# ecmwf-ifs/dwarf-p-cloudsc2-tl-ad

Measured on AMD Instinct MI355X. Metric: CLOUDSC2 NL columns/sec (fp64, NLEV=137), higher is better.
Workload: dtype f64

## Files before the change

### dwarf_p_cloudsc2_tl_ad_amd/__init__.py

```python
from . import binding
from .binding import (Cloudsc2Error, Params, adjoint_verdict, default_params, device_available, get_math_mode,
                      set_math_mode, taylor_verdict)
from .state import (Cloudsc2State, bytes_per_column, ceta_from_table, column_range, nblocks_of, random_table,
                    state_from_table, synthetic_table, validate_l1)
from .driver import (DeviceState, FlatFields, ResidentState, cloudsc_driver, cloudsc_driver_ad, cloudsc_driver_tl,
                     run_state)
from .autograd import PARAM_NAMES, Cloudsc2Outputs, cloudsc2, param_jacobian, satur
```

### dwarf_p_cloudsc2_tl_ad_amd/binding.py

```python
from __future__ import annotations

import ctypes as C
import os

import numpy as np

CLOUDSC2_MAX_NLEV = 200
CLOUDSC2_EINVAL, CLOUDSC2_ENODEVICE, CLOUDSC2_ETLWRONG = -1, -2, -3

_HERE = os.path.dirname(os.path.abspath(__file__))
SINGLE = os.environ.get("CLOUDSC2_PRECISION", "double").strip().lower() in ("single", "sp", "f32", "fp32", "float32")
REAL = np.float32 if SINGLE else np.float64
REAL_BYTES = 4 if SINGLE else 8
c_real = C.c_float if SINGLE else C.c_double
LIB_PATH = os.environ.get("CLOUDSC2_LIB") or os.path.join(_HERE, "csrc", "libcloudsc2_hip_sp.so" if SINGLE else "libcloudsc2_hip.so")


def torch_real():
    import torch

    return torch.float32 if SINGLE else torch.float64


class Cloudsc2Error(RuntimeError):
# ... 17 lines not shown

    def set_ceta(self, ceta) -> "Params":
        ceta = np.asarray(ceta, dtype=np.float64)
        if ceta.size > CLOUDSC2_MAX_NLEV:
            raise ValueError("nlev exceeds CLOUDSC2_MAX_NLEV")
        self.nlev = int(ceta.size)
        for k, v in enumerate(ceta):
            self.ceta[k] = float(v)
        return self

    def ceta_array(self) -> np.ndarray:
        return np.array(self.ceta[: self.nlev], dtype=np.float64)


class Field(C.Structure):

    _fields_ = [("ptr", C.c_void_p), ("block_stride", C.c_longlong)]


IN_NAMES = ("paph", "pap", "q", "qsat", "t", "l", "i", "lude", "lu", "mfu", "mfd", "gtent", "gtenq", "gtenl",
            "gteni", "supsat")
OUT_NAMES = ("tent", "tenq", "tenl", "teni", "clc", "fplsl", "fplsn", "fhpsl", "fhpsn", "covptot")
PARAM_NAMES = ("rkconv", "rclcrit", "rlptrc", "rpecons")


class Inputs(C.Structure):

    _fields_ = [(n, Field) for n in IN_NAMES]


class Outputs(C.Structure):

    _fields_ = [(n, Field) for n in OUT_NAMES]


def _load() -> C.CDLL:
    if not os.path.exists(LIB_PATH):
        raise ImportError(
            f"{LIB_PATH} not found: the HIP library has not been built (run `python -c 'import __graft_entry__ as g; "
            "g.build()'` or `make -C dwarf_p_cloudsc2_tl_ad_amd/csrc`). There is no CPU fallback.")
    try:
        import torch
    except ImportError:
        pass
    lib = C.CDLL(LIB_PATH)
    dp = C.POINTER(C.c_double)
    rp = C.POINTER(c_real)
    pp = C.POINTER(Params)
    lib.cloudsc2_real_bytes.restype = C.c_int
    if lib.cloudsc2_real_bytes() != REAL_BYTES:
        raise ImportError(f"{LIB_PATH} works on {lib.cloudsc2_real_bytes()}-byte reals, CLOUDSC2_PRECISION asks for {REAL_BYTES}")
    lib.cloudsc2_params_default.argtypes = [pp]
    lib.cloudsc2_params_default.restype = None
    lib.cloudsc2_last_error.restype = C.c_char_p
    lib.cloudsc2_device_available.restype = C.c_int
    lib.cloudsc2_set_math_mode.argtypes = [C.c_int]
    lib.cloudsc2_set_math_mode.restype = None
    lib.cloudsc2_get_math_mode.restype = C.c_int
    lib.cloudsc2_nl_launch.argtypes = [pp, C.c_double, C.c_int, C.c_int, C.c_int, C.POINTER(Inputs), C.POINTER(Outputs),
                                       Field, C.c_double, C.c_void_p]
    lib.cloudsc2_satur_launch.argtypes = [pp, C.c_int, C.c_int, C.c_int, Field, Field, Field, C.c_void_p]
    lib.cloudsc2_tl_launch.argtypes = [pp, C.c_double, C.c_int, C.c_int, C.c_int, C.POINTER(Inputs), C.POINTER(Outputs),
                                       C.POINTER(Inputs), C.POINTER(Outputs), C.c_void_p]
    lib.cloudsc2_tl_launch_self.argtypes = [pp, C.c_double, C.c_int, C.c_int, C.c_int, C.POINTER(Inputs), C.POINTER(Outputs), C.c_double,
                                            C.POINTER(Outputs), C.c_void_p, C.c_void_p]
    lib.cloudsc2_ad_launch_reverse_norms.argtypes = [pp, C.c_double, C.c_int, C.c_int, C.c_int, C.POINTER(Inputs), C.POINTER(Outputs),
# ... 23 lines not shown
    lib.cloudsc2_par_work_doubles.argtypes = [C.c_int, C.c_int, C.POINTER(C.c_longlong)]
    lib.cloudsc2_par_work_doubles.restype = C.c_int
    lib.cloudsc2_tl_launch_par.argtypes = [pp, C.c_double, C.c_int, C.c_int, C.c_int, C.c_int, C.POINTER(Inputs), C.POINTER(Inputs),
                                           C.POINTER(C.c_double), C.POINTER(Outputs), C.c_void_p]
    lib.cloudsc2_tl_launch_par.restype = C.c_int
    lib.cloudsc2_vjp_launch_par.argtypes = [pp, C.c_double, C.c_int, C.c_int, C.c_int, C.c_int, C.POINTER(Inputs), C.POINTER(Outputs),
                                            C.POINTER(Inputs), C.POINTER(Outputs), C.c_void_p, C.c_void_p, C.c_void_p, C.c_void_p]
    lib.cloudsc2_vjp_launch_par.restype = C.c_int
    lib.cloudsc2_tl_launch_parjac.argtypes = [pp, C.c_double, C.c_int, C.c_int, C.c_int, C.POINTER(Inputs), C.POINTER(Outputs), C.c_void_p]
    lib.cloudsc2_tl_launch_parjac.restype = C.c_int
    lib.cloudsc2_batch_max.argtypes = []
    lib.cloudsc2_batch_max.restype = C.c_int
    lib.cloudsc2_tl_launch_batch.argtypes = [pp, C.c_double, C.c_int, C.c_int, C.c_int, C.POINTER(Inputs), C.c_int,
                                             C.POINTER(Inputs), C.POINTER(Outputs), C.c_void_p]
    lib.cloudsc2_tl_launch_batch.restype = C.c_int
    lib.cloudsc2_vjp_launch_batch.argtypes = [pp, C.c_double, C.c_int, C.c_int, C.c_int, C.POINTER(Inputs), C.POINTER(Outputs), C.c_int,
                                              C.POINTER(Inputs), C.POINTER(Outputs), C.c_void_p, C.c_void_p]
    lib.cloudsc2_vjp_launch_batch.restype = C.c_int
    lib.cloudsc2_taylor_sums_launch.argtypes = [C.c_int, C.c_int, C.c_int, C.POINTER(Outputs), C.POINTER(Outputs),
                                                C.POINTER(Outputs), C.c_double, C.c_void_p, C.c_void_p]
    lib.cloudsc2_taylor_sweep_work_doubles.argtypes = [C.c_int, C.c_int, C.POINTER(C.c_longlong)]
    lib.cloudsc2_taylor_sweep_work_doubles.restype = C.c_int
    lib.cloudsc2_taylor_sweep_launch.argtypes = [pp, C.c_double, C.c_int, C.c_int, C.c_int, C.c_int, C.POINTER(Inputs), C.POINTER(Outputs),
                                                 C.POINTER(Outputs), C.c_void_p, C.c_void_p, C.c_void_p]
    lib.cloudsc2_taylor_sweep_launch.restype = C.c_int
    lib.cloudsc2_adjoint_norms_launch.argtypes = [C.c_int, C.c_int, C.c_int, C.POINTER(Inputs), C.POINTER(Field),
                                                  C.POINTER(Outputs), C.POINTER(Inputs), C.c_void_p, C.c_void_p,
                                                  C.c_void_p]
    host18 = [rp] * 18
    lib.cloudsc2_nl_run.argtypes = [pp, C.c_int, C.c_int, C.c_int, C.c_double] + host18 + [dp]
    lib.cloudsc2_tl_taylor_run.argtypes = [pp, C.c_int, C.c_int, C.c_int, C.c_double] + host18 + [dp, dp]
    lib.cloudsc2_ad_symmetry_run.argtypes = [pp, C.c_int, C.c_int, C.c_int, C.c_double] + host18 + [dp, dp]
    lib.cloudsc2_release_workspace.restype = None
    lib.cloudsc2_state_create.argtypes = [C.c_int, C.c_int, C.c_int, C.POINTER(C.c_void_p)]
    lib.cloudsc2_state_destroy.argtypes = [C.c_void_p]
    lib.cloudsc2_state_destroy.restype = None
    lib.cloudsc2_state_field.argtypes = [C.c_void_p, C.c_int, C.POINTER(Field)]
    lib.cloudsc2_state_blocking.argtypes = [C.c_void_p, C.POINTER(C.c_int), C.POINTER(C.c_int)]
    lib.cloudsc2_state_blocking.restype = C.c_int
    lib.cloudsc2_state_expand.argtypes = [C.c_void_p, C.c_int, rp, C.c_int, C.c_int, C.c_longlong]
    lib.cloudsc2_state_upload.argtypes = [C.c_void_p] + host18
    lib.cloudsc2_state_download.argtypes = [C.c_void_p] + [rp] * 7
    lib.cloudsc2_state_nl.argtypes = [C.c_void_p, pp, C.c_double, C.c_int, dp]
    lib.cloudsc2_state_tl_taylor.argtypes = [C.c_void_p, pp, C.c_double, dp, dp]
    lib.cloudsc2_state_ad_symmetry.argtypes = [C.c_void_p, pp, C.c_double, dp, dp]
    lib.cloudsc2_state_validate.argtypes = [C.c_void_p, C.c_int, C.c_int, rp, C.c_int, C.c_int, C.c_longlong, dp]
    for name in ("cloudsc2_state_create", "cloudsc2_state_field", "cloudsc2_state_expand", "cloudsc2_state_upload",
                 "cloudsc2_state_download", "cloudsc2_state_nl", "cloudsc2_state_tl_taylor", "cloudsc2_state_ad_symmetry",
                 "cloudsc2_state_validate"):
        getattr(lib, name).restype = C.c_int
    lib.cloudsc2_device_malloc.argtypes = [C.POINTER(C.c_void_p), C.c_size_t]
    lib.cloudsc2_device_free.argtypes = [C.c_void_p]
    lib.cloudsc2_device_malloc_info.argtypes = [C.POINTER(C.c_int), dp, dp, dp]
    lib.cloudsc2_device_malloc_info.restype = None
    lib.cloudsc2_device_malloc_counts.argtypes = [C.POINTER(C.c_longlong), C.POINTER(C.c_longlong)]
    lib.cloudsc2_device_malloc_counts.restype = None
    lib.cloudsc2_pace_plan.argtypes = [C.c_longlong, C.c_longlong, C.POINTER(C.c_int), C.POINTER(C.c_int), C.POINTER(C.c_int)]
    lib.cloudsc2_pace_plan.restype = C.c_int
    lib.cloudsc2_simd_population.argtypes = [C.c_longlong, C.c_int, C.c_longlong, C.c_int, C.POINTER(C.c_int), C.POINTER(C.c_int)]
    lib.cloudsc2_simd_population.restype = C.c_int
    lib.cloudsc2_dispatch_probe.argtypes = [C.POINTER(C.c_longlong), C.POINTER(C.c_longlong)]
    lib.cloudsc2_dispatch_probe.restype = C.c_int
    lib.cloudsc2_pace_probe.argtypes = [C.c_int, C.POINTER(C.c_longlong), C.POINTER(C.c_longlong)]
    lib.cloudsc2_pace_probe.restype = C.c_int
    lib.cloudsc2_synthetic_table.argtypes = [C.c_int, C.c_int, C.c_double, C.c_double, C.c_double] + [C.POINTER(C.c_double)] * 12
    lib.cloudsc2_synthetic_table.restype = C.c_int
# ... 6 lines not shown
    lib.cloudsc2_device_probe.argtypes = [C.c_void_p, C.c_size_t, C.c_int, C.c_int, dp]
    lib.cloudsc2_device_probe.restype = C.c_int
    lib.cloudsc2_device_malloc_state.argtypes = [C.POINTER(C.c_void_p), C.c_size_t, C.c_int, C.c_int, C.c_int]
    lib.cloudsc2_device_malloc_state.restype = C.c_int
    lib.cloudsc2_taylor_verdict.argtypes = [dp, C.POINTER(C.c_int)]
    lib.cloudsc2_adjoint_verdict.argtypes = [C.c_double]
    expand_args = [rp, C.c_int, C.c_int, C.c_longlong, C.c_int, C.c_int, C.c_int, C.c_longlong, Field]
    lib.cloudsc2_expand_launch.argtypes = expand_args + [C.c_void_p]
    lib.cloudsc2_validate_workspace_doubles.restype = C.c_int
    lib.cloudsc2_validate_launch.argtypes = expand_args + [dp, dp, C.c_void_p]
    lib.cloudsc2_expand_offsets.argtypes = [C.c_int, C.c_longlong, C.c_longlong, C.c_int, C.c_int, C.POINTER(C.c_longlong),
                                            C.POINTER(C.c_int)]
    lib.cloudsc2_expand_offsets.restype = None
    lib.cloudsc2_validate_relerr.argtypes = [C.c_double, C.c_double, C.POINTER(C.c_int), C.POINTER(C.c_int)]
    lib.cloudsc2_validate_relerr.restype = C.c_double
    lib.cloudsc2_validate_format.argtypes = [C.c_char_p, C.c_int, dp, C.c_longlong, C.c_char_p, C.c_int]
    lib.cloudsc2_validate_header.argtypes = [C.c_char_p, C.c_int]
    for name in ("cloudsc2_expand_launch", "cloudsc2_validate_launch", "cloudsc2_validate_format", "cloudsc2_validate_header",
                 "cloudsc2_nl_launch", "cloudsc2_satur_launch", "cloudsc2_tl_launch", "cloudsc2_ad_launch",
                 "cloudsc2_taylor_sums_launch", "cloudsc2_adjoint_norms_launch", "cloudsc2_nl_run",
                 "cloudsc2_tl_taylor_run", "cloudsc2_ad_symmetry_run", "cloudsc2_taylor_verdict",
                 "cloudsc2_adjoint_verdict", "cloudsc2_device_malloc", "cloudsc2_device_free"):
        getattr(lib, name).restype = C.c_int
    return lib


lib = _load()

EXPORTED = ("cloudsc2_params_default", "cloudsc2_last_error", "cloudsc2_device_available", "cloudsc2_current_device", "cloudsc2_set_math_mode",
            "cloudsc2_get_math_mode", "cloudsc2_real_bytes", "cloudsc2_nl_launch",
            "cloudsc2_satur_launch", "cloudsc2_satur_lin_launch", "cloudsc2_tl_launch_satur", "cloudsc2_vjp_launch_satur", "cloudsc2_par_work_doubles", "cloudsc2_tl_launch_par", "cloudsc2_vjp_launch_par", "cloudsc2_tl_launch_parjac", "cloudsc2_tl_launch", "cloudsc2_tl_launch_self", "cloudsc2_ad_launch", "cloudsc2_ad_launch_assign",
            "cloudsc2_ad_launch_forward", "cloudsc2_ad_launch_reverse", "cloudsc2_vjp_launch", "cloudsc2_batch_max", "cloudsc2_tl_launch_batch", "cloudsc2_vjp_launch_batch", "cloudsc2_ad_launch_reverse_norms", "cloudsc2_taylor_sums_launch",
            "cloudsc2_taylor_sweep_work_doubles", "cloudsc2_taylor_sweep_launch", "cloudsc2_adjoint_norms_launch", "cloudsc2_nl_run", "cloudsc2_tl_taylor_run", "cloudsc2_ad_symmetry_run",
            "cloudsc2_release_workspace", "cloudsc2_taylor_verdict", "cloudsc2_adjoint_verdict",
            "cloudsc2_expand_launch", "cloudsc2_validate_workspace_doubles", "cloudsc2_validate_launch",
            "cloudsc2_expand_offsets", "cloudsc2_validate_relerr", "cloudsc2_validate_format", "cloudsc2_validate_header",
            "cloudsc2_device_malloc", "cloudsc2_device_free", "cloudsc2_device_malloc_info", "cloudsc2_device_malloc_counts", "cloudsc2_pace_plan", "cloudsc2_simd_population", "cloudsc2_dispatch_probe", "cloudsc2_pace_probe", "cloudsc2_device_prepare", "cloudsc2_device_rules", "cloudsc2_kernel_occupancy", "cloudsc2_device_probe", "cloudsc2_device_malloc_state",
            "cloudsc2_state_create", "cloudsc2_state_destroy", "cloudsc2_state_field", "cloudsc2_state_blocking", "cloudsc2_state_expand",
            "cloudsc2_state_upload", "cloudsc2_state_download", "cloudsc2_state_nl", "cloudsc2_state_tl_taylor",
            "cloudsc2_state_ad_symmetry", "cloudsc2_state_validate", "cloudsc2_synthetic_table")

F_FULL = {"PT": 0, "PQ": 1, "PAP": 2, "PAPH": 3, "PLU": 4, "PLUDE": 5, "PMFU": 6, "PMFD": 7, "PA": 8, "PSUPSAT": 9, "PCOVPTOT": 10,
          "PFPLSL": 11, "PFPLSN": 12, "PFHPSL": 13, "PFHPSN": 14, "QSAT": 15}
F_CML_T, F_LOC_T, F_PCLV_QL = 16, 24, 32


def check(rc: int) -> None:
    if rc != 0:
        raise Cloudsc2Error(rc, (lib.cloudsc2_last_error() or b"").decode())


class DeviceBuffer:

    def __init__(self, nbytes: int, state_geom=None):
        p = C.c_void_p()
        if state_geom is None:
            check(lib.cloudsc2_device_malloc(C.byref(p), int(nbytes)))
        else:
            check(lib.cloudsc2_device_malloc_state(C.byref(p), int(nbytes), *[int(x) for x in state_geom]))
        self.ptr, self.nbytes = int(p.value or 0), int(nbytes)
        self.__cuda_array_interface__ = {"shape": (self.nbytes,), "typestr": "|u1", "data": (self.ptr, False), "version": 2}

    def __del__(self):
        if getattr(self, "ptr", 0):
            lib.cloudsc2_device_free(C.c_void_p(self.ptr))
            self.ptr = 0

# ... 133 lines not shown
```

### dwarf_p_cloudsc2_tl_ad_amd/csrc/cloudsc2_driver.hip

```cpp

#include <thread>
#include "cloudsc2_host.hpp"

using namespace cloudsc2;

namespace {


__global__ void __launch_bounds__(256)
scale_planes_kernel(real_t* dst, long long dst_stride, const real_t* src, long long src_stride, long long plane, long long nblocks,
                    real_t factor) {
  long long i = (long long)blockIdx.x * blockDim.x + threadIdx.x;
  if (i >= plane * nblocks) return;
  long long ibl = i / plane, r = i - ibl * plane;
  dst[ibl * dst_stride + r] = src[ibl * src_stride + r] * factor;
}

__global__ void __launch_bounds__(256)
reblock_kernel(const real_t* __restrict__ src, int np_src, long long stride_src, real_t* __restrict__ dst, int np_dst,
               long long stride_dst, long long nrows, long long ncopy, long long nzero) {
  const long long total = nrows * nzero;
  for (long long e = (long long)blockIdx.x * blockDim.x + threadIdx.x; e < total; e += (long long)gridDim.x * blockDim.x) {
    const long long row = e / nzero, g = e - row * nzero;
    const long long bd = g / np_dst, jd = g - bd * np_dst;
    real_t v = 0;
    if (g < ncopy) {
      const long long bs = g / np_src, js = g - bs * np_src;
      v = src[bs * stride_src + row * np_src + js];
    }
    dst[bd * stride_dst + row * np_dst + jd] = v;
  }
}

constexpr size_t kAlignReals = 256 / sizeof(real_t);
size_t r32(size_t n) { return (n + kAlignReals - 1) & ~(kAlignReals - 1); }
// ... 213 lines not shown
                            &out.covptot};
  for (int k = 0; k < 16; ++k) *fi[k] = fld(base + k * plane, stride);
  for (int k = 0; k < 10; ++k) *fo[k] = fld(base + (16 + k) * plane, stride);
}

size_t flat_in_reals(long long ncols_pad, int nlev) { return 15 * r32((size_t)ncols_pad * nlev) + r32((size_t)ncols_pad * (nlev + 1)); }
size_t flat_out_reals(long long ncols_pad, int nlev) { return 6 * r32((size_t)ncols_pad * nlev) + 4 * r32((size_t)ncols_pad * (nlev + 1)); }

struct Timer {
  hipEvent_t a = nullptr, b = nullptr;
  Timer() = default;
  Timer(const Timer&) = delete;
  Timer& operator=(const Timer&) = delete;
  ~Timer() {
    if (a) (void)hipEventDestroy(a);
    if (b) (void)hipEventDestroy(b);
  }
  int start(hipStream_t st) {
    HIP_TRY(hipEventCreate(&a));
    HIP_TRY(hipEventCreate(&b));
    HIP_TRY(hipEventRecord(a, st));
    return 0;
  }
  int stop(hipStream_t st, double* ms) {
    HIP_TRY(hipEventRecord(b, st));
    HIP_TRY(hipEventSynchronize(b));
    float f = 0;
    HIP_TRY(hipEventElapsedTime(&f, a, b));
    if (ms) *ms = f;
    return 0;
  }
};

struct SlabResources {
  hipStream_t s_up = nullptr, s_k = nullptr;
  std::vector<hipEvent_t> ev;
  SlabResources() = default;
  SlabResources(const SlabResources&) = delete;
  SlabResources& operator=(const SlabResources&) = delete;
  ~SlabResources() {
    for (auto e : ev) if (e) (void)hipEventDestroy(e);
    if (s_up) (void)hipStreamDestroy(s_up);
    if (s_k) (void)hipStreamDestroy(s_k);
  }
  int create(size_t nevents) {
    HIP_TRY(hipStreamCreateWithFlags(&s_up, hipStreamNonBlocking));
    HIP_TRY(hipStreamCreateWithFlags(&s_k, hipStreamNonBlocking));
    ev.assign(nevents, nullptr);
    for (auto& e : ev) HIP_TRY(hipEventCreate(&e));
    return 0;
  }
};

HostState host_view(const HostState& h, long long b0, const DevState& d) {
  const long long S = d.S, H = d.H;
  HostState v = h;
  v.pt += b0 * S; v.pq += b0 * S; v.b_cml += b0 * 8 * S; v.b_loc += b0 * 8 * S; v.pap += b0 * S; v.paph += b0 * H;
  v.plu += b0 * S; v.plude += b0 * S; v.pmfu += b0 * S; v.pmfd += b0 * S; v.pa += b0 * S; v.pclv += b0 * 5 * S;
  v.psupsat += b0 * S; v.pcovptot += b0 * S; v.pfplsl += b0 * H; v.pfplsn += b0 * H; v.pfhpsl += b0 * H; v.pfhpsn += b0 * H;
  return v;
}
DevState dev_view(const DevState& d, long long b0, long long nb) {
  const long long S = d.S, H = d.H;
  DevState v = d;
  v.pt += b0 * S; v.pq += b0 * S; v.b_cml += b0 * 8 * S; v.b_loc += b0 * 8 * S; v.pap += b0 * S; v.paph += b0 * H;
  v.plu += b0 * S; v.plude += b0 * S; v.pmfu += b0 * S; v.pmfd += b0 * S; v.pa += b0 * S; v.pclv += b0 * 5 * S;
  v.psupsat += b0 * S; v.pcovptot += b0 * S; v.pfplsl += b0 * H; v.pfplsn += b0 * H; v.pfhpsl += b0 * H; v.pfhpsn += b0 * H;
  v.qsat += b0 * S;
  v.nblocks = nb;
  return v;
}

int upload_slab_sync(const HostState& h, const DevState& d, long long ncols, int nlev, hipStream_t st) {
  int rc = upload(h, d, ncols, nlev, st);
  if (rc) return rc;
  HIP_TRY(hipStreamSynchronize(st));
  return 0;
}

int nl_run_slabs(const cloudsc2_params* prm, double ptsphy, int nproma, int nlev, int ngptot, const Geom& g, const HostState& h,
                 const DevState& d, double* kernel_ms) {
  const long long nb = d.nblocks;
  const long long slab_blocks = std::max<long long>(1, 16384 / nproma);
  const long long nslabs = (nb + slab_blocks - 1) / slab_blocks;
  int device = 0;
  HIP_TRY(hipGetDevice(&device));
  SlabResources res;
  {
    const int rc_res = res.create((size_t)(2 * nslabs));
    if (rc_res) return rc_res;
  }
  const hipStream_t s_up = res.s_up, s_k = res.s_k;
  const std::vector<hipEvent_t>& ev = res.ev;

  std::atomic<long long> uploaded{0};
  std::atomic<int> up_rc{0};
  std::string up_err;
  auto slab_cols = [&](long long i, long long& b0, long long& nbs, long long& active) {
    b0 = i * slab_blocks;
    nbs = std::min(slab_blocks, nb - b0);
    active = std::min<long long>(nbs * nproma, (long long)ngptot - b0 * nproma);
  };
  std::thread uploader([&] {
    if (hipSetDevice(device) != hipSuccess) { up_rc = CLOUDSC2_EINVAL; up_err = "hipSetDevice failed in the upload thread"; return; }
    for (long long i = 0; i < nslabs && up_rc == 0; ++i) {
      long long b0, nbs, active;
      slab_cols(i, b0, nbs, active);
      int rc = upload_slab_sync(host_view(h, b0, d), dev_view(d, b0, nbs), nbs * nproma, nlev, s_up);
      if (rc) { up_err = g_err; up_rc = rc; return; }
      uploaded.store(i + 1, std::memory_order_release);
    }
  });

  int rc = 0;
  for (long long i = 0; i < nslabs && rc == 0; ++i) {
    while (uploaded.load(std::memory_order_acquire) <= i && up_rc == 0) std::this_thread::yield();
    if (up_rc != 0) break;
    long long b0, nbs, active;
    slab_cols(i, b0, nbs, active);
    const DevState dv = dev_view(d, b0, nbs);
    cloudsc2_inputs in; cloudsc2_outputs out;
    traj_blocks(dv, nproma, nlev, false, in, out);
    if (hipEventRecord(ev[2 * i], s_k) != hipSuccess) { rc = fail(CLOUDSC2_EINVAL, "hipEventRecord failed"); break; }
    rc = cloudsc2_nl_launch(prm, ptsphy, nproma, nlev, (int)active, &in, &out, fld(dv.b_loc + 7LL * nproma * nlev, 8 * dv.S), 0.0, s_k);
    if (rc) break;
    if (hipEventRecord(ev[2 * i + 1], s_k) != hipSuccess) { rc = fail(CLOUDSC2_EINVAL, "hipEventRecord failed"); break; }
    rc = download(host_view(h, b0, d), dv, nbs * nproma, nlev, s_k, nproma, active);
  }
  uploader.join();
  if (rc == 0 && up_rc != 0) rc = fail(up_rc, up_err.c_str());
  const hipError_t e_sync = hipStreamSynchronize(s_k);
  if (rc == 0 && e_sync != hipSuccess) rc = fail(CLOUDSC2_EINVAL, hipGetErrorString(e_sync));
  if (rc == 0 && kernel_ms) {
    double total = 0.0;
    for (long long i = 0; i < nslabs; ++i) {
      float f = 0.f;
      if (hipEventElapsedTime(&f, ev[2 * i], ev[2 * i + 1]) == hipSuccess) total += f;
    }
    *kernel_ms = total;
  }
  (void)g;
  return rc;
}

}

extern "C" {

void cloudsc2_release_workspace(void) {
  std::lock_guard<std::mutex> lock(g_arena_mutex);
  g_arena.release();
}

int cloudsc2_nl_run(const cloudsc2_params* prm, int nproma, int nlev, int ngptot, double ptsphy, const cloudsc2_real* pt,
                    const cloudsc2_real* pq, const cloudsc2_real* b_cml, cloudsc2_real* b_loc, const cloudsc2_real* pap, const cloudsc2_real* paph,
                    const cloudsc2_real* plu, const cloudsc2_real* plude, const cloudsc2_real* pmfu, const cloudsc2_real* pmfd, cloudsc2_real* pa,
                    const cloudsc2_real* pclv, const cloudsc2_real* psupsat, cloudsc2_real* pcovptot, cloudsc2_real* pfplsl, cloudsc2_real* pfplsn,
                    cloudsc2_real* pfhpsl, cloudsc2_real* pfhpsn, double* kernel_ms) {
  Geom g;
  int rc = check_geom(prm, nproma, nlev, ngptot, g);
  if (rc) return rc;
  std::lock_guard<std::mutex> lock(g_arena_mutex);
  const ProbeFn probe = state_probe(nproma, nlev, ngptot);
  if ((rc = g_arena.reserve(state_reals(g.ncols_pad, nlev), &probe, kPlaceOnRequest))) return rc;
  DevState d;
  state_take(g_arena, d, g.ncols_pad, nproma, nlev);
  HostState h = {pt, pq, b_cml, b_loc, pap, paph, plu, plude, pmfu, pmfd, pa, pclv, psupsat, pcovptot, pfplsl, pfplsn, pfhpsl, pfhpsn};
  return nl_run_slabs(prm, ptsphy, nproma, nlev, ngptot, g, h, d, kernel_ms);
}

}
namespace {

size_t taylor_nsums(int ngptot, int nproma_stat) { return (size_t)(((long long)ngptot + nproma_stat - 1) / nproma_stat) * 10 * 2 * 10; }
size_t taylor_ws_reals(long long ncols_pad, int nproma, int nlev, int ngptot, int nproma_stat) {
  (void)nproma;
  const size_t nsums = taylor_nsums(ngptot, nproma_stat);
  return std::max(flat_in_reals(ncols_pad, nlev) + flat_out_reals(ncols_pad, nlev), pair_reals(ncols_pad, nlev)) +
         r32((size_t)(10 * kTaylorLambdas + 10) * (size_t)ncols_pad * kF64) + r32(nsums * kF64);
}
size_t adjoint_ws_reals(long long ncols_pad, int nlev) {
  const size_t ncol = (size_t)ncols_pad;
  return std::max(flat_in_reals(ncols_pad, nlev) + flat_out_reals(ncols_pad, nlev), pair_reals(ncols_pad, nlev)) + r32(ncol * nlev) +
         r32(3 * ncol * kF64) + r32(32 * kF64);
}

int taylor_compute(const cloudsc2_params* prm_in, const Geom& g, int nproma, int nlev, int ngptot, double ptsphy, const DevState& d,
                   Arena& ws, double znormg[10], double* kernel_ms, hipStream_t st, int nproma_stat) {
  const long long nblocks_stat = ((long long)ngptot + nproma_stat - 1) / nproma_stat;
  const size_t nsums = taylor_nsums(ngptot, nproma_stat);
  cloudsc2_inputs inc;
  cloudsc2_outputs tlo;
  pair_take(ws, g.ncols_pad, nproma, nlev, inc, tlo);
  (void)inc;
  double* colsum = ws.take_f64((size_t)(10 * kTaylorLambdas + 10) * (size_t)g.ncols_pad);
  double* sums = ws.take_f64(nsums);
  int rc;
  cloudsc2_inputs in; cloudsc2_outputs out;
  traj_blocks(d, nproma, nlev, true, in, out);
  cloudsc2_params prm_call = *prm_in;
  if (prm_call.math_mode == 0) prm_call.math_mode = 2;
// ... 399 lines not shown
```

### dwarf_p_cloudsc2_tl_ad_amd/driver.py

```python
from __future__ import annotations

import ctypes as C

import numpy as np

from . import binding as B
from .state import PLANE_A, PLANE_Q, PLANE_QI, PLANE_QL, PLANE_QV, PLANE_T, Cloudsc2State, nblocks_of

_dp = C.POINTER(C.c_double)
_rp = C.POINTER(B.c_real)


def _ptr(a: np.ndarray):
    if a.dtype != B.REAL or not a.flags["C_CONTIGUOUS"]:
        raise ValueError(f"state arrays must be C-contiguous {np.dtype(B.REAL).name}")
    return a.ctypes.data_as(_rp)


def _host_args(prm: B.Params, nproma, nlev, ngptot, ptsphy, arrays):
    return [C.byref(prm), int(nproma), int(nlev), int(ngptot), float(ptsphy)] + [_ptr(a) for a in arrays]


def cloudsc_driver(prm: B.Params, numomp, nproma, nlev, ngptot, ngptotg, ptsphy, pt, pq, tendency_cml, tendency_loc, pap,
                   paph, plu, plude, pmfu, pmfd, pa, pclv, psupsat, pcovptot, pfplsl, pfplsn, pfhpsl, pfhpsn) -> float:
    del numomp, ngptotg
    ms = C.c_double(0.0)
    arrays = [pt, pq, tendency_cml, tendency_loc, pap, paph, plu, plude, pmfu, pmfd, pa, pclv, psupsat, pcovptot, pfplsl,
              pfplsn, pfhpsl, pfhpsn]
    B.check(B.lib.cloudsc2_nl_run(*_host_args(prm, nproma, nlev, ngptot, ptsphy, arrays), C.byref(ms)))
    return ms.value


def cloudsc_driver_tl(prm: B.Params, numomp, nproma, nlev, ngptot, ngptotg, ptsphy, pt, pq, tendency_cml, tendency_loc,
                      pap, paph, plu, plude, pmfu, pmfd, pa, pclv, psupsat, pcovptot, pfplsl, pfplsn, pfhpsl, pfhpsn):
    del numomp, ngptotg
    ms = C.c_double(0.0)
    zn = (C.c_double * 10)()
    arrays = [pt, pq, tendency_cml, tendency_loc, pap, paph, plu, plude, pmfu, pmfd, pa, pclv, psupsat, pcovptot, pfplsl,
              pfplsn, pfhpsl, pfhpsn]
    B.check(B.lib.cloudsc2_tl_taylor_run(*_host_args(prm, nproma, nlev, ngptot, ptsphy, arrays), zn, C.byref(ms)))
    znormg = np.array(zn[:], dtype=np.float64)
    ok, itest = B.taylor_verdict(znormg)
    return znormg, ok, itest, ms.value


def cloudsc_driver_ad(prm: B.Params, numomp, nproma, nlev, ngptot, ngptotg, ptsphy, pt, pq, tendency_cml, tendency_loc,
                      pap, paph, plu, plude, pmfu, pmfd, pa, pclv, psupsat, pcovptot, pfplsl, pfplsn, pfhpsl, pfhpsn):
    del numomp, ngptotg
    ms = C.c_double(0.0)
    zn = C.c_double(0.0)
    arrays = [pt, pq, tendency_cml, tendency_loc, pap, paph, plu, plude, pmfu, pmfd, pa, pclv, psupsat, pcovptot, pfplsl,
              pfplsn, pfhpsl, pfhpsn]
    B.check(B.lib.cloudsc2_ad_symmetry_run(*_host_args(prm, nproma, nlev, ngptot, ptsphy, arrays), C.byref(zn), C.byref(ms)))
    return zn.value, B.adjoint_verdict(zn.value), ms.value


def run_state(prm: B.Params, st: Cloudsc2State, which: str = "nl"):
    fn = {"nl": cloudsc_driver, "tl": cloudsc_driver_tl, "ad": cloudsc_driver_ad}[which]
    return fn(prm, 1, st.nproma, st.nlev, st.ngptot, st.ngptot, st.ptsphy, *st.driver_arrays())


def _fld(t, offset_elems: int, stride: int) -> B.Field:
    f = B.Field()
    f.ptr = t.data_ptr() + B.REAL_BYTES * offset_elems
    f.block_stride = stride
    return f


class FlatFields:

    NPLANES = len(B.IN_NAMES) + len(B.OUT_NAMES)

    def __init__(self, kind: str, nb: int, nlev: int, nproma: int, device, zero: bool = True, _views=None, _arena=None):
        self.kind = kind
        names = B.IN_NAMES if kind == "in" else B.OUT_NAMES
        half = {"paph"} if kind == "in" else {"fplsl", "fplsn", "fhpsl", "fhpsn"}
        if _views is not None:
            buf, first = _views
            self.buf = buf
            self.t = {n: buf[:, first + k, : nlev + (1 if n in half else 0), :] for k, n in enumerate(names)}
        else:
            shapes = {n: (nb, nlev + (1 if n in half else 0), nproma) for n in names}
            arena = _arena or B.DeviceArena(B.DeviceArena.size_of(shapes.values(), B.REAL_BYTES), device)
            self.t = {n: arena.take(shp, zero=zero) for n, shp in shapes.items()}
        self.nlev, self.nproma = nlev, nproma

    @classmethod
# ... 335 lines not shown
```

### include/cloudsc2_hip.h

```cpp
#ifndef CLOUDSC2_HIP_H
#define CLOUDSC2_HIP_H

#ifdef __cplusplus
extern "C" {
#endif

#ifdef CLOUDSC2_SINGLE
typedef float cloudsc2_real;
#else
typedef double cloudsc2_real;
#endif

#define CLOUDSC2_MAX_NLEV 200

#define CLOUDSC2_EINVAL    (-1)
#define CLOUDSC2_ENODEVICE (-2)
#define CLOUDSC2_ETLWRONG  (-3)

typedef struct cloudsc2_params {
  double rg, rd, rcpd, retv, rlvtt, rlstt, rlmlt, rtt;
  double r2es, r3les, r3ies, r4les, r4ies, r5les, r5ies, r5alvcp, r5alscp,
         ralvdcp, ralsdcp, rtwat, rtice, rtwat_rtice_r, rvtmp2;
  double rclcrit, rkconv, rlmin, rpecons;
  double rlptrc;
// ... 128 lines not shown
                                double* sums, void* stream);

int cloudsc2_taylor_sweep_work_doubles(int nproma, int ngptot, long long* n);
int cloudsc2_taylor_sweep_launch(const cloudsc2_params* prm, double ptsphy, int nproma, int nlev, int ngptot, int nproma_stat,
                                 const cloudsc2_inputs* in, const cloudsc2_outputs* out, const cloudsc2_outputs* tl,
                                 double* work, double* sums, void* stream);

int cloudsc2_adjoint_norms_launch(int nproma, int nlev, int ngptot, const cloudsc2_inputs* traj_in,
                                  const cloudsc2_field* qsat, const cloudsc2_outputs* y,
                                  const cloudsc2_inputs* x_adj, double* norms, double* blockmax, void* stream);

int cloudsc2_nl_run(const cloudsc2_params* prm, int nproma, int nlev, int ngptot, double ptsphy,
                    const cloudsc2_real* pt, const cloudsc2_real* pq, const cloudsc2_real* b_cml, cloudsc2_real* b_loc,
                    const cloudsc2_real* pap, const cloudsc2_real* paph, const cloudsc2_real* plu, const cloudsc2_real* plude,
                    const cloudsc2_real* pmfu, const cloudsc2_real* pmfd, cloudsc2_real* pa, const cloudsc2_real* pclv,
                    const cloudsc2_real* psupsat, cloudsc2_real* pcovptot, cloudsc2_real* pfplsl, cloudsc2_real* pfplsn,
                    cloudsc2_real* pfhpsl, cloudsc2_real* pfhpsn, double* kernel_ms);

int cloudsc2_tl_taylor_run(const cloudsc2_params* prm, int nproma, int nlev, int ngptot, double ptsphy,
                           const cloudsc2_real* pt, const cloudsc2_real* pq, const cloudsc2_real* b_cml, cloudsc2_real* b_loc,
                           const cloudsc2_real* pap, const cloudsc2_real* paph, const cloudsc2_real* plu, const cloudsc2_real* plude,
                           const cloudsc2_real* pmfu, const cloudsc2_real* pmfd, cloudsc2_real* pa, const cloudsc2_real* pclv,
                           const cloudsc2_real* psupsat, cloudsc2_real* pcovptot, cloudsc2_real* pfplsl, cloudsc2_real* pfplsn,
                           cloudsc2_real* pfhpsl, cloudsc2_real* pfhpsn, double znormg[10], double* kernel_ms);

int cloudsc2_ad_symmetry_run(const cloudsc2_params* prm, int nproma, int nlev, int ngptot, double ptsphy,
                             const cloudsc2_real* pt, const cloudsc2_real* pq, const cloudsc2_real* b_cml, cloudsc2_real* b_loc,
                             const cloudsc2_real* pap, const cloudsc2_real* paph, const cloudsc2_real* plu, const cloudsc2_real* plude,
                             const cloudsc2_real* pmfu, const cloudsc2_real* pmfd, cloudsc2_real* pa, const cloudsc2_real* pclv,
                             const cloudsc2_real* psupsat, cloudsc2_real* pcovptot, cloudsc2_real* pfplsl, cloudsc2_real* pfplsn,
                             cloudsc2_real* pfhpsl, cloudsc2_real* pfhpsn, double* znormg, double* kernel_ms);

void cloudsc2_release_workspace(void);

typedef struct cloudsc2_state cloudsc2_state;
enum {
  CLOUDSC2_F_PT = 0, CLOUDSC2_F_PQ, CLOUDSC2_F_PAP, CLOUDSC2_F_PAPH, CLOUDSC2_F_PLU, CLOUDSC2_F_PLUDE, CLOUDSC2_F_PMFU,
  CLOUDSC2_F_PMFD, CLOUDSC2_F_PA, CLOUDSC2_F_PSUPSAT, CLOUDSC2_F_PCOVPTOT,
  CLOUDSC2_F_PFPLSL, CLOUDSC2_F_PFPLSN, CLOUDSC2_F_PFHPSL, CLOUDSC2_F_PFHPSN, CLOUDSC2_F_QSAT,
  CLOUDSC2_F_CML_T = 16,
  CLOUDSC2_F_LOC_T = 24,
  CLOUDSC2_F_PCLV_QL = 32
};
int cloudsc2_state_create(int nproma, int nlev, int ngptot, cloudsc2_state** state);
void cloudsc2_state_destroy(cloudsc2_state* state);
int cloudsc2_state_field(const cloudsc2_state* state, int field, cloudsc2_field* f);
int cloudsc2_state_blocking(const cloudsc2_state* state, int* nproma_device, int* nproma_caller);
int cloudsc2_state_expand(cloudsc2_state* state, int field, const cloudsc2_real* table, int klon, int period, long long start);
int cloudsc2_state_upload(cloudsc2_state* state,
                          const cloudsc2_real* pt, const cloudsc2_real* pq, const cloudsc2_real* b_cml, cloudsc2_real* b_loc,
                          const cloudsc2_real* pap, const cloudsc2_real* paph, const cloudsc2_real* plu, const cloudsc2_real* plude,
                          const cloudsc2_real* pmfu, const cloudsc2_real* pmfd, cloudsc2_real* pa, const cloudsc2_real* pclv,
                          const cloudsc2_real* psupsat, cloudsc2_real* pcovptot, cloudsc2_real* pfplsl, cloudsc2_real* pfplsn,
                          cloudsc2_real* pfhpsl, cloudsc2_real* pfhpsn);
int cloudsc2_state_download(cloudsc2_state* state, cloudsc2_real* b_loc, cloudsc2_real* pa, cloudsc2_real* pcovptot,
                            cloudsc2_real* pfplsl, cloudsc2_real* pfplsn, cloudsc2_real* pfhpsl, cloudsc2_real* pfhpsn);
int cloudsc2_state_nl(cloudsc2_state* state, const cloudsc2_params* prm, double ptsphy, int repeats, double* kernel_ms);
int cloudsc2_state_tl_taylor(cloudsc2_state* state, const cloudsc2_params* prm, double ptsphy, double znormg[10], double* kernel_ms);
int cloudsc2_state_ad_symmetry(cloudsc2_state* state, const cloudsc2_params* prm, double ptsphy, double* znormg, double* kernel_ms);
int cloudsc2_state_validate(cloudsc2_state* state, int field, int ndim, const cloudsc2_real* ref_table, int klon, int period,
                            long long start, double stats[5]);

int cloudsc2_synthetic_table(int klon, int nlev, double rd, double rv, double rtt, double* pt, double* pq, double* pap, double* paph,
                             double* plu, double* plude, double* pmfu, double* pmfd, double* pql, double* pqi, double* tend_t,
                             double* tend_q);

// ... 21 lines not shown
```

Baseline: 207.5 million.

## Pipeline NL slabs across upload, kernel and download streams with persistent workers

Restructures the slab pipeline in the NL host run. Upload, kernel and download now run on three prioritized streams linked by events, instead of each upload being synchronised on the host and downloads sharing the kernel stream. Upload and download are driven by persistent worker threads using condition variables in place of a spinning yield loop. Streams and events are cached globally across calls, and an optional per-slab timeline probe is added. This is meant to overlap host-to-device copies, compute and device-to-host copies and to cut per-call setup cost. In exchange it adds global mutable state and more threading complexity.

```diff
diff --git a/dwarf_p_cloudsc2_tl_ad_amd/__init__.py b/dwarf_p_cloudsc2_tl_ad_amd/__init__.py
--- a/dwarf_p_cloudsc2_tl_ad_amd/__init__.py
+++ b/dwarf_p_cloudsc2_tl_ad_amd/__init__.py
@@ -4,5 +4,5 @@
 from .state import (Cloudsc2State, bytes_per_column, ceta_from_table, column_range, nblocks_of, random_table,
                     state_from_table, synthetic_table, validate_l1)
 from .driver import (DeviceState, FlatFields, ResidentState, cloudsc_driver, cloudsc_driver_ad, cloudsc_driver_tl,
-                     run_state)
+                     nl_timeline, run_state)
 from .autograd import PARAM_NAMES, Cloudsc2Outputs, cloudsc2, param_jacobian, satur
diff --git a/dwarf_p_cloudsc2_tl_ad_amd/binding.py b/dwarf_p_cloudsc2_tl_ad_amd/binding.py
--- a/dwarf_p_cloudsc2_tl_ad_amd/binding.py
+++ b/dwarf_p_cloudsc2_tl_ad_amd/binding.py
@@ -73,6 +73,13 @@
 class Outputs(C.Structure):
 
     _fields_ = [(n, Field) for n in OUT_NAMES]
+
+
+class SlabTimes(C.Structure):
+
+    _fields_ = [(n, C.c_double) for n in ("host_up_begin", "host_up_end", "host_launch_begin", "host_launch_end", "host_down_begin",
+                                          "host_down_end", "dev_up_begin", "dev_up_end", "dev_kernel_begin", "dev_kernel_end",
+                                          "dev_down_begin", "dev_down_end")]
 
 
 def _load() -> C.CDLL:
@@ -162,6 +169,8 @@
     lib.cloudsc2_tl_taylor_run.argtypes = [pp, C.c_int, C.c_int, C.c_int, C.c_double] + host18 + [dp, dp]
     lib.cloudsc2_ad_symmetry_run.argtypes = [pp, C.c_int, C.c_int, C.c_int, C.c_double] + host18 + [dp, dp]
     lib.cloudsc2_release_workspace.restype = None
+    lib.cloudsc2_nl_timeline.argtypes = [C.c_int, C.POINTER(SlabTimes), C.c_int, C.POINTER(C.c_int)]
+    lib.cloudsc2_nl_timeline.restype = C.c_int
     lib.cloudsc2_state_create.argtypes = [C.c_int, C.c_int, C.c_int, C.POINTER(C.c_void_p)]
     lib.cloudsc2_state_destroy.argtypes = [C.c_void_p]
     lib.cloudsc2_state_destroy.restype = None
@@ -234,7 +243,7 @@
             "cloudsc2_satur_launch", "cloudsc2_satur_lin_launch", "cloudsc2_tl_launch_satur", "cloudsc2_vjp_launch_satur", "cloudsc2_par_work_doubles", "cloudsc2_tl_launch_par", "cloudsc2_vjp_launch_par", "cloudsc2_tl_launch_parjac", "cloudsc2_tl_launch", "cloudsc2_tl_launch_self", "cloudsc2_ad_launch", "cloudsc2_ad_launch_assign",
             "cloudsc2_ad_launch_forward", "cloudsc2_ad_launch_reverse", "cloudsc2_vjp_launch", "cloudsc2_batch_max", "cloudsc2_tl_launch_batch", "cloudsc2_vjp_launch_batch", "cloudsc2_ad_launch_reverse_norms", "cloudsc2_taylor_sums_launch",
             "cloudsc2_taylor_sweep_work_doubles", "cloudsc2_taylor_sweep_launch", "cloudsc2_adjoint_norms_launch", "cloudsc2_nl_run", "cloudsc2_tl_taylor_run", "cloudsc2_ad_symmetry_run",
-            "cloudsc2_release_workspace", "cloudsc2_taylor_verdict", "cloudsc2_adjoint_verdict",
+            "cloudsc2_release_workspace", "cloudsc2_nl_timeline", "cloudsc2_taylor_verdict", "cloudsc2_adjoint_verdict",
             "cloudsc2_expand_launch", "cloudsc2_validate_workspace_doubles", "cloudsc2_validate_launch",
             "cloudsc2_expand_offsets", "cloudsc2_validate_relerr", "cloudsc2_validate_format", "cloudsc2_validate_header",
             "cloudsc2_device_malloc", "cloudsc2_device_free", "cloudsc2_device_malloc_info", "cloudsc2_device_malloc_counts", "cloudsc2_pace_plan", "cloudsc2_simd_population", "cloudsc2_dispatch_probe", "cloudsc2_pace_probe", "cloudsc2_device_prepare", "cloudsc2_device_rules", "cloudsc2_kernel_occupancy", "cloudsc2_device_probe", "cloudsc2_device_malloc_state",
diff --git a/dwarf_p_cloudsc2_tl_ad_amd/csrc/cloudsc2_driver.hip b/dwarf_p_cloudsc2_tl_ad_amd/csrc/cloudsc2_driver.hip
--- a/dwarf_p_cloudsc2_tl_ad_amd/csrc/cloudsc2_driver.hip
+++ b/dwarf_p_cloudsc2_tl_ad_amd/csrc/cloudsc2_driver.hip
@@ -1,6 +1,9 @@
 
+#include <chrono>
+#include <condition_variable>
 #include <thread>
 #include "cloudsc2_host.hpp"
+#include "cloudsc2_slabs.hpp"
 
 using namespace cloudsc2;
 
@@ -280,26 +283,6 @@
   }
 };
 
-struct SlabResources {
-  hipStream_t s_up = nullptr, s_k = nullptr;
-  std::vector<hipEvent_t> ev;
-  SlabResources() = default;
-  SlabResources(const SlabResources&) = delete;
-  SlabResources& operator=(const SlabResources&) = delete;
-  ~SlabResources() {
-    for (auto e : ev) if (e) (void)hipEventDestroy(e);
-    if (s_up) (void)hipStreamDestroy(s_up);
-    if (s_k) (void)hipStreamDestroy(s_k);
-  }
-  int create(size_t nevents) {
-    HIP_TRY(hipStreamCreateWithFlags(&s_up, hipStreamNonBlocking));
-    HIP_TRY(hipStreamCreateWithFlags(&s_k, hipStreamNonBlocking));
-    ev.assign(nevents, nullptr);
-    for (auto& e : ev) HIP_TRY(hipEventCreate(&e));
-    return 0;
-  }
-};
-
 HostState host_view(const HostState& h, long long b0, const DevState& d) {
   const long long S = d.S, H = d.H;
   HostState v = h;
@@ -319,76 +302,207 @@
   return v;
 }
 
-int upload_slab_sync(const HostState& h, const DevState& d, long long ncols, int nlev, hipStream_t st) {
-  int rc = upload(h, d, ncols, nlev, st);
-  if (rc) return rc;
-  HIP_TRY(hipStreamSynchronize(st));
-  return 0;
-}
-
-int nl_run_slabs(const cloudsc2_params* prm, double ptsphy, int nproma, int nlev, int ngptot, const Geom& g, const HostState& h,
-                 const DevState& d, double* kernel_ms) {
-  const long long nb = d.nblocks;
-  const long long slab_blocks = std::max<long long>(1, 16384 / nproma);
-  const long long nslabs = (nb + slab_blocks - 1) / slab_blocks;
-  int device = 0;
-  HIP_TRY(hipGetDevice(&device));
-  SlabResources res;
-  {
-    const int rc_res = res.create((size_t)(2 * nslabs));
-    if (rc_res) return rc_res;
-  }
-  const hipStream_t s_up = res.s_up, s_k = res.s_k;
-  const std::vector<hipEvent_t>& ev = res.ev;
-
-  std::atomic<long long> uploaded{0};
-  std::atomic<int> up_rc{0};
-  std::string up_err;
-  auto slab_cols = [&](long long i, long long& b0, long long& nbs, long long& active) {
-    b0 = i * slab_blocks;
-    nbs = std::min(slab_blocks, nb - b0);
-    active = std::min<long long>(nbs * nproma, (long long)ngptot - b0 * nproma);
+class Worker {
+ public:
+  Worker() : th_([this] { loop(); }) {}
+  Worker(const Worker&) = delete;
+  Worker& operator=(const Worker&) = delete;
+  ~Worker() {
+    { std::lock_guard<std::mutex> l(m_); quit_ = true; }
+    cv_.notify_all();
+    th_.join();
+  }
+  void post(std::function<void()> job) {
+    { std::lock_guard<std::mutex> l(m_); job_ = std::move(job); busy_ = true; }
+    cv_.notify_all();
+  }
+  void wait() {
+    std::unique_lock<std::mutex> l(m_);
+    cv_.wait(l, [this] { return !busy_; });
+  }
+
+ private:
+  void loop() {
+    std::unique_lock<std::mutex> l(m_);
+    for (;;) {
+      cv_.wait(l, [this] { return quit_ || job_; });
+      if (quit_) return;
+      std::function<void()> job = std::move(job_);
+      job_ = nullptr;
+      l.unlock();
+      job();
+      l.lock();
+      busy_ = false;
+      cv_.notify_all();
+    }
+  }
+  std::mutex m_;
+  std::condition_variable cv_;
+  std::function<void()> job_;
+  bool busy_ = false, quit_ = false;
+  std::thread th_;
+};
+
+struct Handoff {
+  std::mutex m;
+  std::condition_variable cv;
+  long long uploaded = 0, launched = 0;
+  int rc = 0;
+  std::string err;
+  void done(long long Handoff::*stage) {
+    { std::lock_guard<std::mutex> l(m); ++(this->*stage); }
+    cv.notify_all();
+  }
+  bool wait_for(long long Handoff::*stage, long long i) {
+    std::unique_lock<std::mutex> l(m);
+    cv.wait(l, [&] { return rc != 0 || this->*stage > i; });
+    return rc == 0;
+  }
+  bool ok() { std::lock_guard<std::mutex> l(m); return rc == 0; }
+  void failed(int code, const std::string& msg) {
+    { std::lock_guard<std::mutex> l(m); if (rc == 0) { rc = code; err = msg; } }
+    cv.notify_all();
+  }
+};
+
+enum SlabEvent { kUpBegin = 0, kUpEnd, kKernelBegin, kKernelEnd, kDownBegin, kDownEnd, kSlabEvents };
+struct SlabPipeline {
+  int device = -1;
+  hipStream_t s_up = nullptr, s_k = nullptr, s_down = nullptr;
+  std::vector<hipEvent_t> ev;
+  Worker up, down;
+  SlabPipeline() = default;
+  SlabPipeline(const SlabPipeline&) = delete;
+  SlabPipeline& operator=(const SlabPipeline&) = delete;
+  ~SlabPipeline() {
+    for (auto e : ev) if (e) (void)hipEventDestroy(e);
+    for (auto s : {s_up, s_k, s_down}) if (s) (void)hipStreamDestroy(s);
+  }
+  int create(int dev) {
+    device = dev;
+    int least = 0, greatest = 0;
+    HIP_TRY(hipDeviceGetStreamPriorityRange(&least, &greatest));
+    HIP_TRY(hipStreamCreateWithPriority(&s_up, hipStreamNonBlocking, greatest));
+    HIP_TRY(hipStreamCreateWithPriority(&s_k, hipStreamNonBlocking, (least + greatest) / 2));
+    HIP_TRY(hipStreamCreateWithPriority(&s_down, hipStreamNonBlocking, least));
+    return 0;
+  }
+  int events_for(long long nslabs) {
+    const size_t need = 1 + (size_t)kSlabEvents * (size_t)nslabs;
+    while (ev.size() < need) {
+      hipEvent_t e = nullptr;
+      HIP_TRY(hipEventCreate(&e));
+      ev.push_back(e);
+    }
+    return 0;
+  }
+  hipEvent_t event(long long slab, SlabEvent k) const { return ev[1 + (size_t)kSlabEvents * (size_t)slab + k]; }
+};
+SlabPipeline* g_pipe = nullptr;
+
+int pipeline_get(long long nslabs, SlabPipeline** out) {
+  int dev = 0;
+  HIP_TRY(hipGetDevice(&dev));
+  if (g_pipe && g_pipe->device != dev) { delete g_pipe; g_pipe = nullptr; }
+  if (!g_pipe) {
+    SlabPipeline* p = new SlabPipeline;
+    const int rc = p->create(dev);
+    if (rc) { delete p; return rc; }
+    g_pipe = p;
+  }
+  const int rc = g_pipe->events_for(nslabs);
+  if (rc) return rc;
+  *out = g_pipe;
+  return 0;
+}
+
+std::atomic<bool> g_timeline_on{false};
+std::mutex g_timeline_mutex;
+std::vector<cloudsc2_slab_times> g_timeline;
+using Clock = std::chrono::steady_clock;
+double ms_since(Clock::time_point t0) { return std::chrono::duration<double, std::milli>(Clock::now() - t0).count(); }
+
+int nl_run_slabs(const cloudsc2_params* prm, double ptsphy, int nproma, int nlev, int ngptot, const HostState& h, const DevState& d,
+                 double* kernel_ms) {
+  const long long nb = d.nblocks, nslabs = slab_count(nb, nproma);
+  SlabPipeline* pp = nullptr;
+  int rc = pipeline_get(nslabs, &pp);
+  if (rc) return rc;
+  SlabPipeline& p = *pp;
+  const bool timed = g_timeline_on.load();
+  std::vector<cloudsc2_slab_times> rows(timed ? (size_t)nslabs : 0);
+  if (timed) HIP_TRY(hipEventRecord(p.ev[0], p.s_up));
+  const Clock::time_point t0 = Clock::now();
+  Handoff ho;
+  auto hip_ok = [&](hipError_t e, const char* what) {
+    if (e == hipSuccess) return true;
+    ho.failed((int)e, std::string(what) + ": " + hipGetErrorString(e));
+    return false;
   };
-  std::thread uploader([&] {
-    if (hipSetDevice(device) != hipSuccess) { up_rc = CLOUDSC2_EINVAL; up_err = "hipSetDevice failed in the upload thread"; return; }
-    for (long long i = 0; i < nslabs && up_rc == 0; ++i) {
-      long long b0, nbs, active;
-      slab_cols(i, b0, nbs, active);
-      int rc = upload_slab_sync(host_view(h, b0, d), dev_view(d, b0, nbs), nbs * nproma, nlev, s_up);
-      if (rc) { up_err = g_err; up_rc = rc; return; }
-      uploaded.store(i + 1, std::memory_order_release);
+
+  p.up.post([&] {
+    if (!hip_ok(hipSetDevice(p.device), "hipSetDevice (upload thread)")) return;
+    for (long long i = 0; i < nslabs && ho.ok(); ++i) {
+      const Slab sl = slab_at(i, nb, nproma, ngptot);
+      if (timed) { rows[i].host_up_begin = ms_since(t0); (void)hipEventRecord(p.event(i, kUpBegin), p.s_up); }
+      const int r = upload(host_view(h, sl.b0, d), dev_view(d, sl.b0, sl.nblocks), sl.nblocks * nproma, nlev, p.s_up);
+      if (r) { ho.failed(r, g_err); return; }
+      if (!hip_ok(hipEventRecord(p.event(i, kUpEnd), p.s_up), "hipEventRecord (upload)")) return;
+      if (timed) rows[i].host_up_end = ms_since(t0);
+      ho.done(&Handoff::uploaded);
     }
   });
-
-  int rc = 0;
-  for (long long i = 0; i < nslabs && rc == 0; ++i) {
-    while (uploaded.load(std::memory_order_acquire) <= i && up_rc == 0) std::this_thread::yield();
-    if (up_rc != 0) break;
-    long long b0, nbs, active;
-    slab_cols(i, b0, nbs, active);
-    const DevState dv = dev_view(d, b0, nbs);
+  p.down.post([&] {
+    if (!hip_ok(hipSetDevice(p.device), "hipSetDevice (download thread)")) return;
+    for (long long i = 0; i < nslabs; ++i) {
+      if (!ho.wait_for(&Handoff::launched, i)) return;
+      const Slab sl = slab_at(i, nb, nproma, ngptot);
+      if (timed) rows[i].host_down_begin = ms_since(t0);
+      if (!hip_ok(hipStreamWaitEvent(p.s_down, p.event(i, kKernelEnd), 0), "hipStreamWaitEvent (download)")) return;
+      if (timed) (void)hipEventRecord(p.event(i, kDownBegin), p.s_down);
+      const int r = download(host_view(h, sl.b0, d), dev_view(d, sl.b0, sl.nblocks), sl.nblocks * nproma, nlev, p.s_down, nproma, sl.active);
+      if (r) { ho.failed(r, g_err); return; }
+      if (timed) { (void)hipEventRecord(p.event(i, kDownEnd), p.s_down); rows[i].host_down_end = ms_since(t0); }
+    }
+  });
+  for (long long i = 0; i < nslabs; ++i) {
+    if (!ho.wait_for(&Handoff::uploaded, i)) break;
+    const Slab sl = slab_at(i, nb, nproma, ngptot);
+    const DevState dv = dev_view(d, sl.b0, sl.nblocks);
     cloudsc2_inputs in; cloudsc2_outputs out;
     traj_blocks(dv, nproma, nlev, false, in, out);
-    if (hipEventRecord(ev[2 * i], s_k) != hipSuccess) { rc = fail(CLOUDSC2_EINVAL, "hipEventRecord failed"); break; }
-    rc = cloudsc2_nl_launch(prm, ptsphy, nproma, nlev, (int)active, &in, &out, fld(dv.b_loc + 7LL * nproma * nlev, 8 * dv.S), 0.0, s_k);
-    if (rc) break;
-    if (hipEventRecord(ev[2 * i + 1], s_k) != hipSuccess) { rc = fail(CLOUDSC2_EINVAL, "hipEventRecord failed"); break; }
-    rc = download(host_view(h, b0, d), dv, nbs * nproma, nlev, s_k, nproma, active);
-  }
-  uploader.join();
-  if (rc == 0 && up_rc != 0) rc = fail(up_rc, up_err.c_str());
-  const hipError_t e_sync = hipStreamSynchronize(s_k);
-  if (rc == 0 && e_sync != hipSuccess) rc = fail(CLOUDSC2_EINVAL, hipGetErrorString(e_sync));
-  if (rc == 0 && kernel_ms) {
+    if (timed) rows[i].host_launch_begin = ms_since(t0);
+    if (!hip_ok(hipStreamWaitEvent(p.s_k, p.event(i, kUpEnd), 0), "hipStreamWaitEvent (kernel)")) break;
+    if (!hip_ok(hipEventRecord(p.event(i, kKernelBegin), p.s_k), "hipEventRecord (kernel)")) break;
+    const int r = cloudsc2_nl_launch(prm, ptsphy, nproma, nlev, (int)sl.active, &in, &out, fld(dv.b_loc + 7LL * nproma * nlev, 8 * dv.S), 0.0, p.s_k);
+    if (r) { ho.failed(r, g_err); break; }
+    if (!hip_ok(hipEventRecord(p.event(i, kKernelEnd), p.s_k), "hipEventRecord (kernel)")) break;
+    if (timed) rows[i].host_launch_end = ms_since(t0);
+    ho.done(&Handoff::launched);
+  }
+  p.up.wait();
+  p.down.wait();
+  for (auto s : {p.s_up, p.s_k, p.s_down}) (void)hip_ok(hipStreamSynchronize(s), "hipStreamSynchronize");
+  if (ho.rc) return fail(ho.rc, ho.err.c_str());
+  if (kernel_ms) {
     double total = 0.0;
     for (long long i = 0; i < nslabs; ++i) {
       float f = 0.f;
-      if (hipEventElapsedTime(&f, ev[2 * i], ev[2 * i + 1]) == hipSuccess) total += f;
+      if (hipEventElapsedTime(&f, p.event(i, kKernelBegin), p.event(i, kKernelEnd)) == hipSuccess) total += f;
     }
     *kernel_ms = total;
   }
-  (void)g;
-  return rc;
+  if (timed) {
+    auto at = [&](long long i, SlabEvent k) { float f = -1.f; return hipEventElapsedTime(&f, p.ev[0], p.event(i, k)) == hipSuccess ? (double)f : -1.0; };
+    for (long long i = 0; i < nslabs; ++i) {
+      rows[i].dev_up_begin = at(i, kUpBegin); rows[i].dev_up_end = at(i, kUpEnd);
+      rows[i].dev_kernel_begin = at(i, kKernelBegin); rows[i].dev_kernel_end = at(i, kKernelEnd);
+      rows[i].dev_down_begin = at(i, kDownBegin); rows[i].dev_down_end = at(i, kDownEnd);
+    }
+    std::lock_guard<std::mutex> lock(g_timeline_mutex);
+    g_timeline = rows;
+  }
+  return 0;
 }
 
 }
@@ -397,7 +511,17 @@
 
 void cloudsc2_release_workspace(void) {
   std::lock_guard<std::mutex> lock(g_arena_mutex);
+  delete g_pipe;
+  g_pipe = nullptr;
   g_arena.release();
+}
+
+int cloudsc2_nl_timeline(int enable, cloudsc2_slab_times* rows, int capacity, int* nslabs) {
+  if (enable >= 0) g_timeline_on.store(enable != 0);
+  std::lock_guard<std::mutex> lock(g_timeline_mutex);
+  if (nslabs) *nslabs = (int)g_timeline.size();
+  if (rows && capacity > 0) std::copy_n(g_timeline.begin(), std::min<size_t>((size_t)capacity, g_timeline.size()), rows);
+  return 0;
 }
 
 int cloudsc2_nl_run(const cloudsc2_params* prm, int nproma, int nlev, int ngptot, double ptsphy, const cloudsc2_real* pt,
@@ -414,7 +538,7 @@
   DevState d;
   state_take(g_arena, d, g.ncols_pad, nproma, nlev);
   HostState h = {pt, pq, b_cml, b_loc, pap, paph, plu, plude, pmfu, pmfd, pa, pclv, psupsat, pcovptot, pfplsl, pfplsn, pfhpsl, pfhpsn};
-  return nl_run_slabs(prm, ptsphy, nproma, nlev, ngptot, g, h, d, kernel_ms);
+  return nl_run_slabs(prm, ptsphy, nproma, nlev, ngptot, h, d, kernel_ms);
 }
 
 }
diff --git a/dwarf_p_cloudsc2_tl_ad_amd/csrc/cloudsc2_slabs.hpp b/dwarf_p_cloudsc2_tl_ad_amd/csrc/cloudsc2_slabs.hpp
--- /dev/null
+++ b/dwarf_p_cloudsc2_tl_ad_amd/csrc/cloudsc2_slabs.hpp
@@ -0,0 +1,24 @@
+#pragma once
+#include <algorithm>
+
+namespace cloudsc2 {
+
+constexpr long long kSlabColumns = 16384;
+
+struct Slab {
+  long long b0;
+  long long nblocks;
+  long long active;
+};
+
+inline long long slab_blocks(int nproma) { return std::max<long long>(1, kSlabColumns / nproma); }
+inline long long slab_count(long long nblocks, int nproma) { return (nblocks + slab_blocks(nproma) - 1) / slab_blocks(nproma); }
+inline Slab slab_at(long long i, long long nblocks, int nproma, long long ngptot) {
+  Slab s;
+  s.b0 = i * slab_blocks(nproma);
+  s.nblocks = std::min(slab_blocks(nproma), nblocks - s.b0);
+  s.active = std::min(s.nblocks * nproma, ngptot - s.b0 * nproma);
+  return s;
+}
+
+}
diff --git a/dwarf_p_cloudsc2_tl_ad_amd/driver.py b/dwarf_p_cloudsc2_tl_ad_amd/driver.py
--- a/dwarf_p_cloudsc2_tl_ad_amd/driver.py
+++ b/dwarf_p_cloudsc2_tl_ad_amd/driver.py
@@ -53,6 +53,15 @@
               pfplsn, pfhpsl, pfhpsn]
     B.check(B.lib.cloudsc2_ad_symmetry_run(*_host_args(prm, nproma, nlev, ngptot, ptsphy, arrays), C.byref(zn), C.byref(ms)))
     return zn.value, B.adjoint_verdict(zn.value), ms.value
+
+
+def nl_timeline(enable: bool | None = None, max_slabs: int = 4096):
+    if enable is not None:
+        B.check(B.lib.cloudsc2_nl_timeline(int(bool(enable)), None, 0, None))
+        return []
+    rows, n = (B.SlabTimes * max_slabs)(), C.c_int(0)
+    B.check(B.lib.cloudsc2_nl_timeline(-1, rows, max_slabs, C.byref(n)))
+    return [{f: getattr(rows[i], f) for f, _ in B.SlabTimes._fields_} for i in range(min(n.value, max_slabs))]
 
 
 def run_state(prm: B.Params, st: Cloudsc2State, which: str = "nl"):
diff --git a/include/cloudsc2_hip.h b/include/cloudsc2_hip.h
--- a/include/cloudsc2_hip.h
+++ b/include/cloudsc2_hip.h
@@ -184,6 +184,12 @@
                              cloudsc2_real* pfhpsl, cloudsc2_real* pfhpsn, double* znormg, double* kernel_ms);
 
 void cloudsc2_release_workspace(void);
+
+typedef struct cloudsc2_slab_times {
+  double host_up_begin, host_up_end, host_launch_begin, host_launch_end, host_down_begin, host_down_end;
+  double dev_up_begin, dev_up_end, dev_kernel_begin, dev_kernel_end, dev_down_begin, dev_down_end;
+} cloudsc2_slab_times;
+int cloudsc2_nl_timeline(int enable, cloudsc2_slab_times* rows, int capacity, int* nslabs);
 
 typedef struct cloudsc2_state cloudsc2_state;
 enum {
```

Result: no change. 206.5 million (-0.5%).
